# chto/linna

Measured on AMD Instinct MI355X. Metric: emulator log-likelihood evals/sec, higher is better.
Workload: dtype f32; 1 GPU; 33-D Gaussian, 4x512 MLP emulator (33->512x4->33), nwalkers=4096 batched log-likelihood per GPU (BASELINE configs[1]); nwalkers_per_gpu=4096, launch=direct launches, parallelism=walkers sharded, 1 rank(s), no data-path collective

## Files before the change

include/linna_hip.h:

```cpp
#ifndef LINNA_HIP_H
#define LINNA_HIP_H
#include <stddef.h>
#include <stdint.h>

#ifdef __cplusplus
extern "C" {
#endif

#define LINNA_ABI_VERSION 12

typedef struct linna_ctx linna_ctx_t;
typedef struct linna_net linna_net_t;
typedef struct linna_logprob linna_logprob_t;
typedef struct linna_graph linna_graph_t;

int linna_abi_version(void);
const char* linna_last_error(void);
#define LINNA_OK 0
#define LINNA_ERR_INVALID (-1)
#define LINNA_ERR_HIP (-2)
#define LINNA_ERR_UNSUPPORTED (-3)
#define LINNA_ERR_INTERNAL (-4)
int linna_debug_raise(int kind);
int linna_ctx_create(int device, linna_ctx_t** out);
// ... 129 lines not shown
                         linna_logprob_t** out);
int linna_logprob_destroy(linna_logprob_t* lp);
int linna_weights_changed(linna_ctx_t* ctx);
#define LINNA_PRECISION_FP32 0
#define LINNA_PRECISION_BF16 1
int linna_logprob_set_precision(linna_logprob_t* lp, int precision);
int linna_logprob_precision(const linna_logprob_t* lp, int* out);
int linna_logprob_set_grad_precision(linna_logprob_t* lp, int precision);
int linna_logprob_grad_precision(const linna_logprob_t* lp, int* out);
int linna_logprob_set_dense_grad(linna_logprob_t* lp, int on);
int linna_logprob_dense_grad(const linna_logprob_t* lp, int* out);
int linna_engine_rows(int rows);
int linna_dense_tri(int mode);
int linna_serve_plain(int on);
int linna_serve_plain_sched(int hand);
int linna_program_plain(const linna_layer_t* layers, int nlayers, int in_size, int rows, int dense_nout);
int linna_logprob_serve_plain(linna_logprob_t* lp, int B, int* out);
int linna_logprob_grad_launches(linna_logprob_t* lp, int B, int* out);
int linna_slice_fusion(int mask);
int linna_program_describe(const linna_layer_t* layers, int nlayers, int in_size, int rows, int dense_nout, char* buf,
                           size_t n);
int linna_program_describe_grad_bf16(const linna_layer_t* layers, int nlayers, int in_size, int rows, char* buf, size_t n);
int linna_program_describe_grad_dense(const linna_layer_t* layers, int nlayers, int in_size, int nout, int tri, int rows,
                                      char* buf, size_t n);
size_t linna_logprob_ws_bytes(const linna_logprob_t* lp, int B, int with_grad);
int linna_logprob_eval(linna_logprob_t* lp, const float* Z, int ldz, int B, void* ws, float* lnP,
                       float* THETA, int ldt, void* stream);
int linna_logprob_eval_if(linna_logprob_t* lp, const float* Z, int ldz, int B, void* ws, float* lnP,
                          float* THETA, int ldt, const int* gate, void* stream);
int linna_logprob_eval_slice_points(linna_logprob_t* lp, const float* coords, int ldc, int ndim, const int* S_idx,
// ... 196 lines not shown
```

linna_amd/_lib.py:

```python
import ctypes as C
import os

import torch

_HERE = os.path.dirname(os.path.abspath(__file__))
LIB_PATH = os.environ.get("LINNA_LIB_PATH") or os.path.join(_HERE, "liblinna_hip.so")
ABI_VERSION = 12
RHAT_BLOCK = 128

c_float_p = C.c_void_p
c_int_p = C.c_void_p


class _Sized(C.Structure):

    def __init__(self, *a, **k):
        C.Structure.__init__(self, *a, **k)
        self.struct_size = C.sizeof(type(self))


def sized_array(cls, n):
    arr = (cls * n)()
    for i in range(n):
        arr[i].struct_size = C.sizeof(cls)
# ... 95 lines not shown
    "linna_gauss_loglike_diag": (_I, [_V, _V, _I, _I, _I, _V, _V, _I, _I, _F, _V, _V]),
    "linna_gauss_loglike_dense": (_I, [_V, _V, _I, _I, _I, _V, _I, _V, _I, _I, _F, _V, _V, _V]),
    "linna_logprob_create": (_I, [_V, _V, C.POINTER(LogprobDesc), _PV]),
    "linna_logprob_destroy": (_I, [_V]),
    "linna_weights_changed": (_I, [_V]),
    "linna_logprob_set_precision": (_I, [_V, _I]),
    "linna_logprob_precision": (_I, [_V, _V]),
    "linna_logprob_set_grad_precision": (_I, [_V, _I]),
    "linna_logprob_grad_precision": (_I, [_V, _V]),
    "linna_logprob_set_dense_grad": (_I, [_V, _I]),
    "linna_logprob_dense_grad": (_I, [_V, _V]),
    "linna_engine_rows": (_I, [_I]),
    "linna_dense_tri": (_I, [_I]),
    "linna_serve_plain": (_I, [_I]),
    "linna_serve_plain_sched": (_I, [_I]),
    "linna_program_plain": (_I, [_V, _I, _I, _I, _I]),
    "linna_logprob_serve_plain": (_I, [_V, _I, _V]),
    "linna_logprob_grad_launches": (_I, [_V, _I, _V]),
    "linna_slice_fusion": (_I, [_I]),
    "linna_net_train_launches": (_I, [_V, _I]),
    "linna_net_set_train_precision": (_I, [_V, _I]),
    "linna_net_train_precision": (_I, [_V, _V]),
    "linna_program_describe": (_I, [_V, _I, _I, _I, _I, _V, C.c_size_t]),
    "linna_program_describe_grad_bf16": (_I, [_V, _I, _I, _I, _V, C.c_size_t]),
    "linna_program_describe_grad_dense": (_I, [_V, _I, _I, _I, _I, _I, _V, C.c_size_t]),
    "linna_logprob_ws_bytes": (_SZ, [_V, _I, _I]),
    "linna_logprob_eval": (_I, [_V, _V, _I, _I, _V, _V, _V, _I, _V]),
    "linna_logprob_grad": (_I, [_V, _V, _I, _I, _V, _V, _V, _I, _V]),
    "linna_logprob_grad_leapfrog": (_I, [_V, _V, _I, _I, _V, _V, _V, _I, _V, _I, _V, _F, _F, _V]),
    "linna_loss_scratch_bytes": (_SZ, [_I, _I]),
# ... 199 lines not shown

def slice_fusion(mask=-1):
    prev = load().linna_slice_fusion(int(mask))
    if prev < 0:
        check(prev)
    return prev


def serve_plain_sched(hand=-1):
    prev = load().linna_serve_plain_sched(int(hand))
    if prev < 0:
        check(prev)
    return prev


def serve_plain(on=-1):
    prev = load().linna_serve_plain(int(on))
    if prev < 0:
        check(prev)
    return prev


def engine_rows(rows=0):
    prev = load().linna_engine_rows(int(rows))
    if prev < 0:
        check(prev)
    return prev
```

linna_amd/csrc/api.hip:

```cpp
#include "common.h"

#include <stdarg.h>
#include <stdio.h>
#include <string.h>
#include <cstring>
#include <string>
#include <vector>
#include <atomic>
#include <new>
#include <stdlib.h>

namespace linna {

static thread_local std::string g_err;

void set_error(const char* fmt, ...) {
    char buf[512];
    va_list ap;
    va_start(ap, fmt);
    vsnprintf(buf, sizeof buf, fmt, ap);
    va_end(ap);
    g_err = buf;
}

// ... 1121 lines not shown
    static float dummy;
    if (dense_nout == -1) return net_stream_describe(ns_grad_kind(layers, nlayers), layers, nlayers, in_size, nullptr, rows, buf, n);
    const int dn_cols = dense_nout < -1 ? -dense_nout : dense_nout;
    NsDense dn{&dummy, (dn_cols + 3) & ~3, nullptr, nullptr, dense_nout < -1 ? 1 : 0, net_stream_dense_tri(-1)};
    if (dn_cols > 0) return net_stream_describe(NS_SERVE_DENSE, layers, nlayers, in_size, &dn, rows, buf, n);
    return net_stream_describe(NS_SERVE, layers, nlayers, in_size, nullptr, rows, buf, n);
} LINNA_CATCH_INT
int linna_serve_plain(int on) try {
    if (on < -1 || on > 1) { set_error("linna_serve_plain: %d (-1 query, 0 or 1)", on); return LINNA_ERR_INVALID; }
    return net_stream_serve_plain(on);
} LINNA_CATCH_INT
int linna_serve_plain_sched(int hand) try {
    if (hand < -1 || hand > 1) { set_error("linna_serve_plain_sched: %d (-1 query, 0 or 1)", hand); return LINNA_ERR_INVALID; }
    return net_stream_serve_plain_sched(hand);
} LINNA_CATCH_INT
int linna_program_plain(const linna_layer_t* layers, int nlayers, int in_size, int rows, int dense_nout) try {
    if (!layers || nlayers < 1) { set_error("program_plain: bad arguments"); return LINNA_ERR_INVALID; }
    TRY(check_layers(layers, nlayers, "program_plain"));
    if (dense_nout != 0) return 0;
    return net_stream_program_plain(NS_SERVE, layers, nlayers, in_size, nullptr, rows) ? 1 : 0;
} LINNA_CATCH_INT
int linna_logprob_serve_plain(linna_logprob_t* lp, int B, int* out) try {
    if (!lp || !out || B < 1) { set_error("logprob_serve_plain: bad arguments"); return LINNA_ERR_INVALID; }
    static float lnP;
    *out = lp_eval_route(lp, false).route == LP_EVAL_ONE &&
           net_stream_takes_plain(lp->kind(), net_layers(lp->net, lp->kind()), lp_output(lp), NsRun{nullptr, 0, B, &lnP}, nullptr, nullptr,
                                  net_stream_rows(B), nullptr);
    return LINNA_OK;
} LINNA_CATCH_INT
int linna_dense_tri(int mode) try {
// ... 740 lines not shown
```

linna_amd/csrc/common.h:

```cpp
#pragma once
#include <hip/hip_runtime.h>
#include <stdint.h>
#include <exception>
#include "../../include/linna_hip.h"


typedef float f32x4 __attribute__((ext_vector_type(4)));
typedef float f32x16 __attribute__((ext_vector_type(16)));

namespace linna {

struct U4 { uint32_t x, y, z, w; };
__device__ __forceinline__ U4 philox4x32_10(U4 c, uint32_t k0, uint32_t k1) {
#pragma unroll
    for (int r = 0; r < 10; ++r) {
        const uint64_t p0 = (uint64_t)0xD2511F53u * c.x;
        const uint64_t p1 = (uint64_t)0xCD9E8D57u * c.z;
        U4 n;
        n.x = (uint32_t)(p1 >> 32) ^ c.y ^ k0;
        n.y = (uint32_t)p1;
        n.z = (uint32_t)(p0 >> 32) ^ c.w ^ k1;
        n.w = (uint32_t)p0;
        c = n;
        k0 += 0x9E3779B9u; k1 += 0xBB67AE85u;
// ... 280 lines not shown
    NS_GRAD_INPUT_DENSE,
};
inline bool ns_kind_full_layers(NsKind k) { return k == NS_SERVE || k == NS_SERVE_DENSE || k == NS_SERVE_BF16; }
struct NsPlan { bool ok; size_t packed_floats; bool grad_ok; const char* why; };
NsPlan net_stream_plan(NsKind kind, const linna_layer_t* layers, int nl, int in_size, const NsDense* dn = nullptr);
int net_stream_rows(int B);
int net_stream_force_rows(int rows);
inline NsKind ns_grad_kind(const linna_layer_t* layers, int nl) { return nl >= 1 && layers[nl - 1].N > 64 ? NS_GRAD_INPUT_WIDE : NS_GRAD_INPUT; }
bool net_stream_grad_fits(const linna_layer_t* layers, int nl, int in_size, int rows);
bool net_stream_grad_dense_fits(const linna_layer_t* layers, int nl, int in_size, const NsDense* dn, int rows);
int launch_net_stream_pack(NsKind kind, const linna_layer_t* layers, int nl, int in_size, float* packed, int rows, const NsDense* dn,
                           hipStream_t s);
int net_stream_describe(NsKind kind, const linna_layer_t* layers, int nl, int in_size, const NsDense* dn, int rows, char* buf, size_t n);
int net_stream_serve_plain(int on);
int net_stream_serve_plain_sched(int hand);
bool net_stream_program_plain(NsKind kind, const linna_layer_t* layers, int nl, int in_size, const NsDense* dn, int rows);
bool net_stream_launch_plain_ok(bool cscale, bool cshift, bool w, bool cexp, bool lnP, bool D, bool TH, bool gate);
struct NsNet { const linna_layer_t* layers; int nl, in_size; };
struct NsInput { int nin; const int* is_flat; const float* a1; const float* a2; const int* lg; const float* xmean; const float* xstd; };
struct NsOutput { const float* cscale; const float* cshift; const float* cpost; const float* cshift2; const float* w; float T; };
struct NsRun { const float* Z; int ldz; int B; float* lnP; const int* gate = nullptr; float* TH = nullptr; int ldt = 0; float* D = nullptr; int ldd = 0; };
struct NsOpBufs { float* y; int ldy; float* t; int ldt; const float* x; int ldx; const float* gate; float* dprev; int ldp; float* dt; int lddt; };
struct NsPost { const float* rows; int n; float scale; float* out; int* step; float* hyper; float b1, b2; };
int launch_net_stream_dx(const NsNet& net, const float* packed, const float* dOUT, int lddo, int B, const NsOpBufs* ops, int with_input,
                         int rows, hipStream_t s, const NsPost* post = nullptr);
struct NsMove {
    float* coords; int ldc; float* logp; const int* S;
    const float* cc; int ldcc; const int* C; int nc;
    unsigned long long seed; const int* step; int step_off; int stream; float a; int* naccept;
    int slice;
// ... 98 lines not shown
```

linna_amd/csrc/net_program.hip:

```cpp
#include "net_program.h"
#include <stdlib.h>
#include <algorithm>
#include <atomic>
#include <cstring>
#include <mutex>
#include <string>
#include <unordered_map>

namespace linna {

size_t NsProgram::lds_for(int rows, bool grad) const {
    size_t b = (size_t)(2 * rows * LD + ((bias_total + 3) & ~3)) * sizeof(float) + 128 + (x0_keep ? 4096 : 0);
#ifdef NS_STAMPS
    b += NS_NW * 32 * 8;
#endif
    return b + (grad ? (size_t)mask_slots * 64 * NS_NW * sizeof(unsigned) : 0);
}

static int ceil16(int k) { return (k + 15) & ~15; }
int ns_seg_steps(const NsSeg& s) {
    if (s.type == NS_WIDE && s.zext < 0) return 2 * s.steps - 60;
    return s.type == NS_WIDE && s.zext > 0 ? s.steps + (s.passes - 1) * s.zext : s.steps * s.passes;
}
static int ns_switch(std::atomic<int>& sw, const char* name, int dflt, bool (*valid)(int)) {
// ... 399 lines not shown
        if (g.type != NS_WIDE && g.type != NS_SPLIT) return false;
        if (g.x0_col || (g.type == NS_WIDE && (g.zext || g.kslice))) return false;
    }
    return true;
}
bool net_stream_program_plain(NsKind kind, const linna_layer_t* layers, int nl, int in_size, const NsDense* dn, int rows) {
    return kind == NS_SERVE && rows == 16 && ns_program_plain(*ns_program(kind, layers, nl, in_size, dn, rows));
}
bool net_stream_launch_plain_ok(bool cscale, bool cshift, bool w, bool cexp, bool lnP, bool D, bool TH, bool gate) {
    return cscale && cshift && w && !cexp && lnP && !D && !TH && !gate;
}
static std::atomic<int> g_serve_plain{1};
int net_stream_serve_plain(int on) { return on < 0 ? g_serve_plain.load() : g_serve_plain.exchange(on ? 1 : 0); }
static std::atomic<int> g_serve_plain_sched{1};
int net_stream_serve_plain_sched(int hand) { return hand < 0 ? g_serve_plain_sched.load() : g_serve_plain_sched.exchange(hand ? 1 : 0); }

int ns_seg_cols(const NsProgram& p, const linna_layer_t* layers, int i) {
    if (p.seg_op[i] >= p.nops) return p.nout;
    const linna_layer_t& l = layers[p.seg_op[i]];
    return p.seg_hidden[i] ? l.C : i < p.nseg_f ? l.N : l.K;
}
NsGates ns_gates(const NsProgram& p, const linna_layer_t* layers, int nl, int rows) {
    NsGates g;
    for (int i = 0; i < NS_SEGCAP; ++i) g.gbit[i] = g.mbit[i] = -1;
    for (int i = 0; i < p.nseg_f; ++i) {
        const int op = p.seg_op[i];
        if (op >= nl || (!p.seg_hidden[i] && op == nl - 1)) continue;
        g.gbit[i] = g.ncols;
        g.ncols += (ns_seg_cols(p, layers, i) + 63) & ~63;
    }
// ... 235 lines not shown
```

linna_amd/csrc/net_stream.hip:

```cpp
#include "net_program.h"
#include <stdlib.h>
#include <type_traits>
#include <cstring>
#include <algorithm>

namespace linna {

typedef __bf16 bf16x8 __attribute__((ext_vector_type(8)));
typedef short s16x4 __attribute__((ext_vector_type(4)));

#ifndef NS_R
#define NS_R 6
#endif
#ifndef NS_PRE
#define NS_PRE 2
#endif
struct NsArgs {
    const float* Z; int ldz; int B; int nin;
    const int* is_flat; const float* a1; const float* a2; const int* lg;
    const float* xmean; const float* xstd;
    const float* packed;
    int G, nseg, LD, kpad0, nout, bias_total;
    int Gstride, nseg_f;
    const float* gscale; float* Gout; int ldg;
    float* hm_p; int hm_ldp; float* hm_q; const float* hm_mass; float hm_ek, hm_ed;
    const float* cscale; const float* cshift; const float* w; float T;
    const float* cpost; const float* cshift2;
    float* lnP; float* D; int ldd; float* TH; int ldt;
    unsigned long long* stamps;
    const int* gate;
    float* gout[NS_SEGCAP]; int gld[NS_SEGCAP]; int gn[NS_SEGCAP];
// ... 179 lines not shown
    constexpr int MOVE = 0, STORE = 0, ROWS = 16;
    constexpr bool GRAD = false, BF = false, EPS = false, PLAIN = true, WOUT = false, DGR = false;
#include "net_stream_body.inc"
}
#if NS_R == 6
#define NS_HAVE_PLACED 1
template <int R>
__global__ __launch_bounds__(64 * NS_NW, 1) void net_stream_placed_kernel(NsArgs a) {
    constexpr int MOVE = 0, STORE = 0, ROWS = 16;
    constexpr bool GRAD = false, BF = false, EPS = false, PLAIN = true, WOUT = false, DGR = false;
#define NS_BODY_HAND
#include "net_stream_body.inc"
#undef NS_BODY_HAND
}
#endif
template <int R, int MOVE, bool GRAD, int STORE, int ROWS, bool BF>
__global__ __launch_bounds__(64 * NS_NW, 1) void net_stream_train_bf16_kernel(NsArgs a) {
    static_assert(BF && GRAD && STORE == 3 && ROWS == 4 && MOVE == 0, "the bf16 training step only");
    constexpr bool EPS = false, PLAIN = false, WOUT = false, DGR = false;
#include "net_stream_body.inc"
}
template <int R, int MOVE, bool GRAD, int STORE, int ROWS, bool BF>
__global__ __launch_bounds__(64 * NS_NW, 1) void net_stream_slice_bf16_kernel(NsArgs a) {
    static_assert(BF && !GRAD && STORE == 0 && MOVE == 2, "the bf16 slice evaluation only");
    constexpr bool EPS = false, PLAIN = false, WOUT = false, DGR = false;
#define NS_BODY_SLICE_BF16
#include "net_stream_body.inc"
#undef NS_BODY_SLICE_BF16
}
template <int R, int MOVE, bool GRAD, int STORE, int ROWS, bool BF>
// ... 46 lines not shown
        }
        for (int ps = 0; ps < p.seg[i].passes; ++ps) {
            a.run_seg[nrun] = i; a.run_pass[nrun] = ps; a.run_first[nrun] = first;
            first += (ps > 0 && p.seg[i].type == NS_WIDE && p.seg[i].zext > 0) ? p.seg[i].zext : p.seg[i].steps; ++nrun;
        }
    }
    a.run_first[nrun] = first; a.nrun = nrun;
    const size_t total = (size_t)NS_NW * p.Gstride * NS_NT * 64 + (size_t)p.bias_total;
    hipLaunchKernelGGL(ns_pack_kernel, dim3((unsigned)((total + 255) / 256)), dim3(256), 0, s, a);
    if (p.side_f4) hipLaunchKernelGGL(ns_pack_side_kernel, dim3((unsigned)((p.side_f4 + 255) / 256)), dim3(256), 0, s, a);
    return check_hip(hipGetLastError(), "net_stream pack launch");
}

typedef void (*NsKernel)(NsArgs);
enum NsVariant { NV_SERVE, NV_STRETCH, NV_SLICE, NV_GRAD_MLP, NV_GRAD2, NV_STORE, NV_DX, NV_TRAIN_FWD, NV_TRAIN_STEP };
enum : unsigned { NF_BF16 = 1, NF_EPS = 2, NF_WIDE = 4, NF_PLAIN = 8, NF_PLACED = 16, NF_DENSE = 32 };
struct NsEntry { NsVariant v; unsigned flags; NsKernel k[3]; const char* what; const char* stamps_lacks; bool attr_set[3]; };
#define NS_ENGINES(K, MOVE, GRAD, STORE, ...) \
    {K<NS_R, MOVE, GRAD, STORE, 16, __VA_ARGS__>, K<NS_R, MOVE, GRAD, STORE, 8, __VA_ARGS__>, K<NS_R, MOVE, GRAD, STORE, 4, __VA_ARGS__>}
static NsEntry ns_table[] = {
    {NV_SERVE, 0, NS_ENGINES(net_stream_kernel, 0, false, 0, false), "net_stream launch"},
    {NV_SERVE, NF_BF16, NS_ENGINES(net_stream_kernel, 0, false, 0, true), "net_stream launch"},
    {NV_SERVE, NF_PLAIN, {net_stream_plain_kernel<NS_R>, nullptr, nullptr}, "net_stream plain launch"},
#ifdef NS_HAVE_PLACED
    {NV_SERVE, NF_PLAIN | NF_PLACED, {net_stream_placed_kernel<NS_R>, nullptr, nullptr}, "net_stream plain launch (hand-placed step)"},
#endif
    {NV_STRETCH, 0, NS_ENGINES(net_stream_kernel, 1, false, 0, false), "net_stream launch"},
    {NV_STRETCH, NF_BF16, NS_ENGINES(net_stream_kernel, 1, false, 0, true), "net_stream launch"},
    {NV_SLICE, 0, NS_ENGINES(net_stream_kernel, 2, false, 0, false), "net_stream launch"},
    {NV_SLICE, NF_BF16, NS_ENGINES(net_stream_slice_bf16_kernel, 2, false, 0, true), "net_stream bf16 slice launch", "bf16 slice evaluation"},
    {NV_GRAD_MLP, 0, NS_ENGINES(net_stream_kernel, 0, true, 0, false), "net_stream launch"},
    {NV_GRAD_MLP, NF_EPS, NS_ENGINES(net_stream_eps_kernel, 0, true, 0, false), "net_stream launch"},
    {NV_GRAD2, 0, NS_ENGINES(net_stream_kernel, 0, true, 2, false), "net_stream launch"},
    {NV_GRAD2, NF_EPS, NS_ENGINES(net_stream_eps_kernel, 0, true, 2, false), "net_stream launch"},
    {NV_GRAD2, NF_WIDE, NS_ENGINES(net_stream_wide_kernel, 0, true, 2, false, false), "net_stream wide-output gradient launch"},
    {NV_GRAD2, NF_WIDE | NF_EPS, NS_ENGINES(net_stream_wide_kernel, 0, true, 2, false, true), "net_stream wide-output gradient launch"},
    {NV_GRAD2, NF_DENSE, NS_ENGINES(net_stream_dense_kernel, 0, true, 2, false, false), "net_stream dense-covariance gradient launch"},
    {NV_GRAD2, NF_DENSE | NF_EPS, NS_ENGINES(net_stream_dense_kernel, 0, true, 2, false, true), "net_stream dense-covariance gradient launch"},
    {NV_GRAD2, NF_BF16, NS_ENGINES(net_stream_grad_bf16_kernel, 0, true, 2, true), "net_stream bf16 gradient launch", "bf16 gradient"},
    {NV_GRAD2, NF_BF16 | NF_EPS, NS_ENGINES(net_stream_eps_bf16_kernel, 0, true, 2, true), "net_stream bf16 gradient launch", "bf16 gradient"},
// ... 226 lines not shown
        a.mv_seed = mv->seed; a.mv_step = mv->step; a.mv_step_off = mv->step_off; a.mv_stream = mv->stream; a.mv_a = mv->a; a.mv_naccept = mv->naccept;
        a.mv_chain = mv->chain; a.mv_lps = mv->lps;
        a.sl_Z0 = mv->sl_Z0; a.sl_L = mv->sl_L; a.sl_R = mv->sl_R; a.sl_Zt = mv->sl_Zt; a.sl_m = mv->sl_m; a.sl_nt = mv->sl_nt;
        a.sl_seed = mv->sl_seed; a.sl_step = mv->sl_step; a.sl_stream = mv->sl_stream; a.sl_flags = mv->sl_flags;
        if (mv->sb) a.sb = *mv->sb;
        return ns_launch_program(mv->slice ? NV_SLICE : NV_STRETCH, fbf, a, r.B, p, rows, s);
    }
    if (bf && gr) { set_error("net_stream: no bf16 gradient"); return LINNA_ERR_UNSUPPORTED; }
    if (bf) return ns_launch_program(NV_SERVE, NF_BF16, a, r.B, p, rows, s);
    if (gr) {
        ns_set_grad(a, *gr);
        return ns_launch_program(NV_GRAD_MLP, a.hm_p && a.hm_eps ? NF_EPS : 0, a, r.B, p, rows, s);
    }
    if (!net_stream_takes_plain(kind, net, out, r, mv, gr, rows, dn)) return ns_launch_program(NV_SERVE, 0, a, r.B, p, rows, s);
    for (int i = 0; i < a.nseg; ++i) a.seg[i].type |= a.seg[i].ncg_log2 << 8;
#ifdef NS_HAVE_PLACED
    if (net_stream_serve_plain_sched(-1)) return ns_launch_program(NV_SERVE, NF_PLAIN | NF_PLACED, a, r.B, p, rows, s);
#endif
    return ns_launch_program(NV_SERVE, NF_PLAIN, a, r.B, p, rows, s);
}

int launch_net_stream_store(const NsNet& net, const float* packed, const float* X, int ldx, int B, const NsOpBufs* ops,
                            const float* cscale, const float* cshift, int rows, hipStream_t s) {
    const NsProgramRef pref = ns_program(NS_STORE, net.layers, net.nl, net.in_size, nullptr, rows);
    const NsProgram& p = *pref;
    if (!p.ok) { set_error("net_stream: network not eligible"); return LINNA_ERR_UNSUPPORTED; }
    NsArgs a = ns_args(p, packed, X, ldx, B, net.in_size, false);
    ns_set_input_ignored(a, X);
    a.cscale = cscale; a.cshift = cshift;
    ns_store_table(a, p, net, ops, 0, p.nseg_f, false);
// ... 106 lines not shown
```

linna_amd/csrc/net_stream_body.inc:

```
    constexpr int NT = NS_NT, NW = NS_NW;
    constexpr int RG = 32;
    constexpr bool SM = ROWS < 16;
    constexpr int RS = SM ? ROWS / 4 : 1;
    constexpr int NQ = SM ? RS : NT;
    constexpr int NACC = SM ? 4 * RS : NT;
#ifdef NS_BODY_SLICE_BF16
    static_assert(BF && !GRAD && STORE == 0 && MOVE == 2, "bf16: the slice evaluation");
#elif defined(NS_BODY_GRAD_BF16)
    static_assert(BF && GRAD && STORE == 2 && MOVE == 0, "bf16: lnP and its gradient in one launch");
#else
    static_assert(!BF || (!GRAD && STORE == 0 && MOVE != 2) || (GRAD && STORE == 3 && MOVE == 0 && ROWS == 4),
                  "bf16: serving, the fused stretch move and the merged training step (4-row engine)");
#endif
    constexpr bool BFT = BF && GRAD && STORE == 3;
    constexpr int AK = BF ? 2 : 1;
    constexpr bool K4 = !SM && !BF && (STORE == 0 || (GRAD && STORE == 2));
    constexpr bool TRB = GRAD && STORE == 3;
    constexpr bool DXE = STORE == 2 || TRB;
    constexpr bool G2 = GRAD && STORE == 2;
    constexpr bool LB = G2;
    constexpr bool LATE_REFILL = true;
#ifdef NS_BODY_HAND
    constexpr bool HAND = true;
    static_assert(PLAIN && !BF && ROWS == 16 && R == 6 && NS_NT == 4 && LATE_REFILL, "the hand-placed step: plain fp32 serving, 16 rows, six slots");
#else
    constexpr bool HAND = false;
#endif
#define NS_HAND_RING \
    "+{v[128:131]}"(Bq[0][0]), "+{v[132:135]}"(Bq[0][1]), "+{v[136:139]}"(Bq[0][2]), "+{v[140:143]}"(Bq[0][3]), \
    "+{v[144:147]}"(Bq[1][0]), "+{v[148:151]}"(Bq[1][1]), "+{v[152:155]}"(Bq[1][2]), "+{v[156:159]}"(Bq[1][3]), \
    "+{v[160:163]}"(Bq[2][0]), "+{v[164:167]}"(Bq[2][1]), "+{v[168:171]}"(Bq[2][2]), "+{v[172:175]}"(Bq[2][3]), \
    "+{v[176:179]}"(Bq[3][0]), "+{v[180:183]}"(Bq[3][1]), "+{v[184:187]}"(Bq[3][2]), "+{v[188:191]}"(Bq[3][3]), \
    "+{v[192:195]}"(Bq[4][0]), "+{v[196:199]}"(Bq[4][1]), "+{v[200:203]}"(Bq[4][2]), "+{v[204:207]}"(Bq[4][3]), \
    "+{v[208:211]}"(Bq[5][0]), "+{v[212:215]}"(Bq[5][1]), "+{v[216:219]}"(Bq[5][2]), "+{v[220:223]}"(Bq[5][3])
#define NS_HAND_A "+{v[224:227]}"(Aq[0][0]), "+{v[228:231]}"(Aq[1][0])
#define NS_HAND_ACC "+{v[232:235]}"(acc[0]), "+{v[236:239]}"(acc[1]), "+{v[240:243]}"(acc[2]), "+{v[244:247]}"(acc[3])
    constexpr bool RNAN = STORE == 1;
    auto relu_f = [](float v) { if constexpr (RNAN) return isnan(v) ? v : fmaxf(v, 0.f); else return fmaxf(v, 0.f); };
    static_assert(ROWS == 16 || ROWS == 8 || ROWS == 4, "rows per workgroup");
    static_assert(R % 2 == 0, "the A double buffer alternates with the ring slot parity");
    extern __shared__ __attribute__((aligned(16))) float smem[];
// ... 309 lines not shown
                asm volatile("global_store_dword %0, %1, off" :: "v"(a.t_xb + (size_t)(row0 + pr) * a.t_ldxb + c), "v"(x) : "memory");
        }
        if constexpr (BF) {
            if (prow) {
                if (c < nin) { const float hi = (float)(__bf16)x; act[pr * LD + c] = hi; act[pr * LD + nin + c] = x - hi; }
                else if (c >= 2 * nin) act[pr * LD + c] = 0.f;
            }
        } else {
            if (prow) act[pr * LD + c] = x;
        }
    }
    __builtin_amdgcn_sched_barrier(0);
#ifdef NS_STAMPS_FINE
    NS_STAMP();
#endif
    NS_PF_ALL(PRE, (LATE_REFILL ? R - 1 : R))
#undef NS_PF_ALL
#undef NS_PF
#pragma unroll
    for (int o = RG / 2; o >= 1; o >>= 1) zz += __shfl_xor(zz, o, 64);
#pragma unroll
    for (int i = 0; i < BMAX; ++i) {
        const int j = tid + i * 64 * NW;
        if (j < nb4) reinterpret_cast<f32x4*>(lbias)[j] = breg[i];
    }
    int* const lsrc = reinterpret_cast<int*>(lbias + ((a.bias_total + 3) & ~3));
    float* const lden = reinterpret_cast<float*>(lsrc + 16);
    if constexpr (STORE == 3) {
        if (prow && pc0 == 0) { lsrc[pr] = zsrc; lden[pr] = zden; }
    }
    float* const lx0 = lden + 16;
// ... 1 lines not shown
    if (a.x0_keep && prow) {
#pragma unroll
        for (int i = 0; i < ZPRE; ++i) {
            const int c = pc0 + i * RG;
            if constexpr (BF) lx0[pr * 64 + c] = c < nin ? act[pr * LD + c] + act[pr * LD + nin + c] : 0.f;
            else lx0[pr * 64 + c] = (c < kpad0) ? act[pr * LD + c] : 0.f;
        }
    }
    }
    asm volatile("s_waitcnt lgkmcnt(0)" ::: "memory");
    __builtin_amdgcn_s_barrier();
    asm volatile("" ::: "memory");
    NS_STAMP();

    if constexpr (HAND) {
#pragma unroll
        for (int t = 0; t < NT; ++t) Bq[R - 1][t] = f32x4{0.f, 0.f, 0.f, 0.f};
        asm volatile("" : NS_HAND_RING :: "memory");
    }
    const uint32_t act_lds = (uint32_t)(uintptr_t)(__attribute__((address_space(3))) void*)act;
    f32x4 acc[NACC];
    f32x4 Aq[2][AK];
    const int sm_arow = (4 * ((lane >> 2) & 3) + (lane & 3)) % ROWS, sm_achunk = lane >> 4;
    int si = 0, pass = 0, P = 0, kleft;
    int s_type, s_steps, s_passes, s_bias, s_dst, s_relu, s_kslice, s_zext, s_ncgl, s_mstore = 0, s_mapply = 0, s_x0col = 0, s_x0n = 0, s_kcl = 0;
    unsigned* const lmask = reinterpret_cast<unsigned*>(lbias + ((a.bias_total + 3) & ~3));
    float lnp_grad = 0.f;
    float* s_gout = nullptr; int s_gld = 0, s_gn = 0;
    const float* s_gmask = nullptr; int s_gmld = 0;
    int s_gbit = -1, s_mbit = -1;
    auto gstore = [&](float* p, float v) { asm volatile("global_store_dword %0, %1, off" :: "v"(p), "v"(v) : "memory"); };
    uint32_t ap;
// ... 52 lines not shown
    auto lds_barrier = [&]() {
        asm volatile("s_waitcnt lgkmcnt(0)" ::: "memory");
        __builtin_amdgcn_s_barrier();
        asm volatile("" ::: "memory");
    };
    if constexpr (PLAIN) {
        asm volatile("" :: "s"(seg_warm));
        plain_take(ka->seg[0]); begin_run(); a_read(Aq[0]); plain_request();
    }
    else {
    load_seg();
    begin_run();
    a_read(Aq[0]);
    }

    auto step = [&](auto Uc, auto Refill) {
        constexpr int U = decltype(Uc)::value;
        constexpr bool refill = decltype(Refill)::value;
        constexpr int RU = LATE_REFILL ? (U + R - 1) % R : U;
        if constexpr (HAND) {
            constexpr int BU = 128 + 16 * U, BR = 128 + 16 * RU, AC = 224 + 4 * (U & 1), AN = 224 + 4 * ((U + 1) & 1);
            constexpr int TW = refill ? 0 : 4 * U;
#define NS_HM(t, s) "v_mfma_f32_16x16x4_f32 v[232+4*" #t ":235+4*" #t "], v[%[ac]+" #s "], v[%[bu]+4*" #t "+" #s "], v[232+4*" #t ":235+4*" #t "]\n\t"
#define NS_HL(t, off) "global_load_dwordx4 v[%[ru]+4*" #t ":%[ru]+4*" #t "+3], %[vo], %[sb] offset:" #off "\n\t"
#define NS_HAND_TEXT(HEAD, L0, L1, L2, L3) HEAD \
            "s_waitcnt lgkmcnt(0)\n\t" \
            "s_waitcnt vmcnt(%[w0])\n\t" \
            NS_HM(0, 0) "ds_read_b128 v[%[an]:%[an]+3], %[ap]\n\t" \
            "s_waitcnt vmcnt(%[w1])\n\t" \
            NS_HM(1, 0) \
            NS_HM(0, 1) L0 \
            NS_HM(1, 1) \
            NS_HM(0, 2) L1 \
            NS_HM(1, 2) \
            NS_HM(0, 3) L2 \
            NS_HM(1, 3) \
            "s_waitcnt vmcnt(%[w2])\n\t" \
            NS_HM(2, 0) L3 \
            "s_waitcnt vmcnt(%[w3])\n\t" \
            NS_HM(3, 0) \
            NS_HM(2, 1) "v_add_u32 %[ap], 64, %[ap]\n\t" \
            NS_HM(3, 1) NS_HM(2, 2) NS_HM(3, 2) NS_HM(2, 3) NS_HM(3, 3)
            if constexpr (refill) {
                const char* const sb = wbase + woff;
#ifdef NS_HAND_PHASE4
#define NS_HAND_HEAD ".p2align 3\n\ts_nop 0\n\t"
#else
#define NS_HAND_HEAD ".p2align 3\n\t"
#endif
                if constexpr (U == 0)
                    asm volatile(NS_HAND_TEXT(NS_HAND_HEAD, NS_HL(0, 0), NS_HL(1, 1024), NS_HL(2, 2048), NS_HL(3, 3072))
                                 : NS_HAND_RING, NS_HAND_A, NS_HAND_ACC, [ap] "+v"(ap)
                                 : [vo] "v"(voff), [sb] "s"(sb), [bu] "n"(BU), [ru] "n"(BR), [ac] "n"(AC), [an] "n"(AN),
                                   [w0] "n"(19), [w1] "n"(18), [w2] "n"(20), [w3] "n"(20) : "memory");
                else
                    asm volatile(NS_HAND_TEXT("", NS_HL(0, 0), NS_HL(1, 1024), NS_HL(2, 2048), NS_HL(3, 3072))
                                 : NS_HAND_RING, NS_HAND_A, NS_HAND_ACC, [ap] "+v"(ap)
                                 : [vo] "v"(voff), [sb] "s"(sb), [bu] "n"(BU), [ru] "n"(BR), [ac] "n"(AC), [an] "n"(AN),
                                   [w0] "n"(19), [w1] "n"(18), [w2] "n"(20), [w3] "n"(20) : "memory");
                wadvance();
            } else {
                asm volatile(NS_HAND_TEXT("", "", "", "", "")
                             : NS_HAND_RING, NS_HAND_A, NS_HAND_ACC, [ap] "+v"(ap)
                             : [bu] "n"(BU), [ac] "n"(AC), [an] "n"(AN),
                               [w0] "n"(19 - TW), [w1] "n"(18 - TW), [w2] "n"(17 - TW), [w3] "n"(16 - TW) : "memory");
            }
#undef NS_HAND_TEXT
#undef NS_HAND_HEAD
#undef NS_HL
#undef NS_HM
        } else {
        if constexpr (BF) asm volatile("s_waitcnt lgkmcnt(0)" : "+v"(Aq[U & 1][0]), "+v"(Aq[U & 1][AK - 1]) :: "memory");
        else asm volatile("s_waitcnt lgkmcnt(0)" : "+v"(Aq[U & 1][0]) :: "memory");
        a_read(Aq[(U + 1) & 1]);
        const f32x4 av = Aq[U & 1][0];
        if constexpr (BF) {
            bf16x8 ab;
#pragma unroll
            for (int e = 0; e < 4; ++e) { ab[e] = (__bf16)Aq[U & 1][0][e]; ab[4 + e] = (__bf16)Aq[U & 1][AK - 1][e]; }
            if constexpr (SM) {
                auto bf_small = [&]() {
                    const s16x4 alo = __builtin_bit_cast(s16x4, __builtin_shufflevector(ab, ab, 0, 1, 2, 3));
                    const s16x4 ahi = __builtin_bit_cast(s16x4, __builtin_shufflevector(ab, ab, 4, 5, 6, 7));
// ... 597 lines not shown
                    take_seg(N2);
                    if constexpr (LB) { s_gbit = ka->gbit[n2i]; s_mbit = ka->mbit[n2i]; s_gn = ka->gn[n2i]; }
                }
            }
            if (si < nseg) {
                begin_run();
                a_read(Aq[(U + 1) & 1]);
                if constexpr (PLAIN) { if (seg_done) plain_request(); }
            }
#ifdef NS_STAMPS_FINE
            if (fine) { asm volatile("s_waitcnt lgkmcnt(0)" ::: "memory"); NS_STAMP(); }
#endif
        }
    };
    using T_ = std::true_type; using F_ = std::false_type;
#define NS_STEP(U, RF) if constexpr (U < R) step(std::integral_constant<int, U>{}, RF{});
    const int ngroups = a.G / R, rem = a.G - ngroups * R;
#pragma unroll 1
    for (int it = 0; it < ngroups; ++it) {
        NS_STEP(0, T_) NS_STEP(1, T_) NS_STEP(2, T_) NS_STEP(3, T_) NS_STEP(4, T_) NS_STEP(5, T_) NS_STEP(6, T_) NS_STEP(7, T_)
    }
#define NS_TAIL(U) if constexpr (U < R - 1) { if (rem > U) step(std::integral_constant<int, U>{}, F_{}); }
    NS_TAIL(0) NS_TAIL(1) NS_TAIL(2) NS_TAIL(3) NS_TAIL(4) NS_TAIL(5) NS_TAIL(6)
#undef NS_STEP
#undef NS_TAIL
    if constexpr (BF) asm volatile("s_waitcnt lgkmcnt(0)" : "+v"(Aq[0][0]), "+v"(Aq[0][AK - 1]), "+v"(Aq[1][0]), "+v"(Aq[1][AK - 1]) :: "memory");
    else asm volatile("s_waitcnt lgkmcnt(0)" : "+v"(Aq[0][0]), "+v"(Aq[1][0]) :: "memory");
    NS_STAMP();

    if constexpr (((STORE == 1 || STORE == 2) && !GRAD) || TRB) { NS_STAMPS_FLUSH(); return; }
    if constexpr (STORE == 3) {
        const float* const F = act + P * ABUF + pr * LD;
        const bool rok = prow && row0 + pr < a.B;
        const float* const Dv = a.u_same ? F : act + (P ^ 1) * ABUF + pr * LD;
        const float* const Uv = a.u_same ? F + a.u_col : F;
        float chi = 0.f;
        for (int c = pc0; c < nout; c += RG) chi += Dv[c] * Uv[c];
#pragma unroll
// ... 125 lines not shown
```

Before: 76.52 million evals/s.

## Ramp the weight-prefetch ring in the hand-placed plain serving kernel head

```diff
diff --git a/include/linna_hip.h b/include/linna_hip.h
--- a/include/linna_hip.h
+++ b/include/linna_hip.h
@@ -167,6 +167,7 @@
 int linna_dense_tri(int mode);
 int linna_serve_plain(int on);
 int linna_serve_plain_sched(int hand);
+int linna_serve_head(int ramp);
 int linna_program_plain(const linna_layer_t* layers, int nlayers, int in_size, int rows, int dense_nout);
 int linna_logprob_serve_plain(linna_logprob_t* lp, int B, int* out);
 int linna_logprob_grad_launches(linna_logprob_t* lp, int B, int* out);
diff --git a/linna_amd/_lib.py b/linna_amd/_lib.py
--- a/linna_amd/_lib.py
+++ b/linna_amd/_lib.py
@@ -133,6 +133,7 @@
     "linna_dense_tri": (_I, [_I]),
     "linna_serve_plain": (_I, [_I]),
     "linna_serve_plain_sched": (_I, [_I]),
+    "linna_serve_head": (_I, [_I]),
     "linna_program_plain": (_I, [_V, _I, _I, _I, _I]),
     "linna_logprob_serve_plain": (_I, [_V, _I, _V]),
     "linna_logprob_grad_launches": (_I, [_V, _I, _V]),
@@ -362,6 +363,13 @@
     return prev
 
 
+def serve_head(ramp=-1):
+    prev = load().linna_serve_head(int(ramp))
+    if prev < 0:
+        check(prev)
+    return prev
+
+
 def serve_plain(on=-1):
     prev = load().linna_serve_plain(int(on))
     if prev < 0:
diff --git a/linna_amd/csrc/api.hip b/linna_amd/csrc/api.hip
--- a/linna_amd/csrc/api.hip
+++ b/linna_amd/csrc/api.hip
@@ -1159,6 +1159,10 @@
     if (hand < -1 || hand > 1) { set_error("linna_serve_plain_sched: %d (-1 query, 0 or 1)", hand); return LINNA_ERR_INVALID; }
     return net_stream_serve_plain_sched(hand);
 } LINNA_CATCH_INT
+int linna_serve_head(int ramp) try {
+    if (ramp < -1 || ramp > 1) { set_error("linna_serve_head: %d (-1 query, 0 or 1)", ramp); return LINNA_ERR_INVALID; }
+    return net_stream_serve_head(ramp);
+} LINNA_CATCH_INT
 int linna_program_plain(const linna_layer_t* layers, int nlayers, int in_size, int rows, int dense_nout) try {
     if (!layers || nlayers < 1) { set_error("program_plain: bad arguments"); return LINNA_ERR_INVALID; }
     TRY(check_layers(layers, nlayers, "program_plain"));
diff --git a/linna_amd/csrc/common.h b/linna_amd/csrc/common.h
--- a/linna_amd/csrc/common.h
+++ b/linna_amd/csrc/common.h
@@ -318,6 +318,7 @@
 int net_stream_describe(NsKind kind, const linna_layer_t* layers, int nl, int in_size, const NsDense* dn, int rows, char* buf, size_t n);
 int net_stream_serve_plain(int on);
 int net_stream_serve_plain_sched(int hand);
+int net_stream_serve_head(int ramp);
 bool net_stream_program_plain(NsKind kind, const linna_layer_t* layers, int nl, int in_size, const NsDense* dn, int rows);
 bool net_stream_launch_plain_ok(bool cscale, bool cshift, bool w, bool cexp, bool lnP, bool D, bool TH, bool gate);
 struct NsNet { const linna_layer_t* layers; int nl, in_size; };
diff --git a/linna_amd/csrc/net_program.hip b/linna_amd/csrc/net_program.hip
--- a/linna_amd/csrc/net_program.hip
+++ b/linna_amd/csrc/net_program.hip
@@ -437,6 +437,8 @@
 int net_stream_serve_plain(int on) { return on < 0 ? g_serve_plain.load() : g_serve_plain.exchange(on ? 1 : 0); }
 static std::atomic<int> g_serve_plain_sched{1};
 int net_stream_serve_plain_sched(int hand) { return hand < 0 ? g_serve_plain_sched.load() : g_serve_plain_sched.exchange(hand ? 1 : 0); }
+static std::atomic<int> g_serve_head{1};
+int net_stream_serve_head(int ramp) { return ramp < 0 ? g_serve_head.load() : g_serve_head.exchange(ramp ? 1 : 0); }
 
 int ns_seg_cols(const NsProgram& p, const linna_layer_t* layers, int i) {
     if (p.seg_op[i] >= p.nops) return p.nout;
diff --git a/linna_amd/csrc/net_stream.hip b/linna_amd/csrc/net_stream.hip
--- a/linna_amd/csrc/net_stream.hip
+++ b/linna_amd/csrc/net_stream.hip
@@ -15,6 +15,22 @@
 #ifndef NS_PRE
 #define NS_PRE 2
 #endif
+#define NS_RAMP_STEPS 3
+constexpr int ns_ring_slots(int pre, int ramped, int tail) { return pre + ramped - tail; }
+constexpr int ns_ring_vmcnt(int pre, int ramped, int tail, int issued, int t) { return 4 * ns_ring_slots(pre, ramped, tail) - 1 - t + issued; }
+static_assert((ns_ring_vmcnt(NS_R - 1, 0, 0, 0, 0) == 19 && ns_ring_vmcnt(NS_R - 1, 0, 0, 0, 1) == 18 &&
+               ns_ring_vmcnt(NS_R - 1, 0, 0, 3, 2) == 20 && ns_ring_vmcnt(NS_R - 1, 0, 0, 4, 3) == 20) || NS_R != 6, "steady step");
+static_assert((ns_ring_vmcnt(NS_PRE, NS_RAMP_STEPS, 0, 0, 0) == 19 && ns_ring_vmcnt(NS_PRE, NS_RAMP_STEPS, 0, 0, 1) == 18 &&
+               ns_ring_vmcnt(NS_PRE, NS_RAMP_STEPS, 0, 3, 2) == 20 && ns_ring_vmcnt(NS_PRE, NS_RAMP_STEPS, 0, 4, 3) == 20) || NS_R != 6 || NS_PRE != 2,
+              "steady step behind the ramp");
+constexpr bool ns_ring_tail_ok(int pre, int ramped) {
+    for (int u = 0; u < 5; ++u)
+        for (int t = 0; t < 4; ++t)
+            if (ns_ring_vmcnt(pre, ramped, u, 0, t) != 19 - 4 * u - t) return false;
+    return true;
+}
+static_assert((ns_ring_tail_ok(NS_R - 1, 0) && ns_ring_tail_ok(NS_PRE, NS_RAMP_STEPS)) || NS_R != 6 || NS_PRE != 2, "tail steps");
+static_assert((4 * ns_ring_slots(NS_PRE, 0, 0) == 8 && 4 * ns_ring_slots(NS_PRE, NS_RAMP_STEPS, 0) == 20) || NS_R != 6 || NS_PRE != 2, "ramp");
 struct NsArgs {
     const float* Z; int ldz; int B; int nin;
     const int* is_flat; const float* a1; const float* a2; const int* lg;
@@ -224,6 +240,19 @@
 #undef NS_BODY_HAND
 }
 #endif
+#if NS_R == 6 && NS_PRE == 2
+#define NS_HAVE_RAMP 1
+template <int R>
+__global__ __launch_bounds__(64 * NS_NW, 1) void net_stream_ramp_kernel(NsArgs a) {
+    constexpr int MOVE = 0, STORE = 0, ROWS = 16;
+    constexpr bool GRAD = false, BF = false, EPS = false, PLAIN = true, WOUT = false, DGR = false;
+#define NS_BODY_HAND
+#define NS_BODY_RAMP
+#include "net_stream_body.inc"
+#undef NS_BODY_RAMP
+#undef NS_BODY_HAND
+}
+#endif
 template <int R, int MOVE, bool GRAD, int STORE, int ROWS, bool BF>
 __global__ __launch_bounds__(64 * NS_NW, 1) void net_stream_train_bf16_kernel(NsArgs a) {
     static_assert(BF && GRAD && STORE == 3 && ROWS == 4 && MOVE == 0, "the bf16 training step only");
@@ -300,7 +329,7 @@
 
 typedef void (*NsKernel)(NsArgs);
 enum NsVariant { NV_SERVE, NV_STRETCH, NV_SLICE, NV_GRAD_MLP, NV_GRAD2, NV_STORE, NV_DX, NV_TRAIN_FWD, NV_TRAIN_STEP };
-enum : unsigned { NF_BF16 = 1, NF_EPS = 2, NF_WIDE = 4, NF_PLAIN = 8, NF_PLACED = 16, NF_DENSE = 32 };
+enum : unsigned { NF_BF16 = 1, NF_EPS = 2, NF_WIDE = 4, NF_PLAIN = 8, NF_PLACED = 16, NF_DENSE = 32, NF_RAMP = 64 };
 struct NsEntry { NsVariant v; unsigned flags; NsKernel k[3]; const char* what; const char* stamps_lacks; bool attr_set[3]; };
 #define NS_ENGINES(K, MOVE, GRAD, STORE, ...) \
     {K<NS_R, MOVE, GRAD, STORE, 16, __VA_ARGS__>, K<NS_R, MOVE, GRAD, STORE, 8, __VA_ARGS__>, K<NS_R, MOVE, GRAD, STORE, 4, __VA_ARGS__>}
@@ -310,6 +339,9 @@
     {NV_SERVE, NF_PLAIN, {net_stream_plain_kernel<NS_R>, nullptr, nullptr}, "net_stream plain launch"},
 #ifdef NS_HAVE_PLACED
     {NV_SERVE, NF_PLAIN | NF_PLACED, {net_stream_placed_kernel<NS_R>, nullptr, nullptr}, "net_stream plain launch (hand-placed step)"},
+#endif
+#ifdef NS_HAVE_RAMP
+    {NV_SERVE, NF_PLAIN | NF_PLACED | NF_RAMP, {net_stream_ramp_kernel<NS_R>, nullptr, nullptr}, "net_stream plain launch (hand-placed step, ramped head)"},
 #endif
     {NV_STRETCH, 0, NS_ENGINES(net_stream_kernel, 1, false, 0, false), "net_stream launch"},
     {NV_STRETCH, NF_BF16, NS_ENGINES(net_stream_kernel, 1, false, 0, true), "net_stream launch"},
@@ -566,6 +598,9 @@
     }
     if (!net_stream_takes_plain(kind, net, out, r, mv, gr, rows, dn)) return ns_launch_program(NV_SERVE, 0, a, r.B, p, rows, s);
     for (int i = 0; i < a.nseg; ++i) a.seg[i].type |= a.seg[i].ncg_log2 << 8;
+#ifdef NS_HAVE_RAMP
+    if (net_stream_serve_plain_sched(-1) && net_stream_serve_head(-1)) return ns_launch_program(NV_SERVE, NF_PLAIN | NF_PLACED | NF_RAMP, a, r.B, p, rows, s);
+#endif
 #ifdef NS_HAVE_PLACED
     if (net_stream_serve_plain_sched(-1)) return ns_launch_program(NV_SERVE, NF_PLAIN | NF_PLACED, a, r.B, p, rows, s);
 #endif
diff --git a/linna_amd/csrc/net_stream_body.inc b/linna_amd/csrc/net_stream_body.inc
--- a/linna_amd/csrc/net_stream_body.inc
+++ b/linna_amd/csrc/net_stream_body.inc
@@ -25,6 +25,12 @@
     static_assert(PLAIN && !BF && ROWS == 16 && R == 6 && NS_NT == 4 && LATE_REFILL, "the hand-placed step: plain fp32 serving, 16 rows, six slots");
 #else
     constexpr bool HAND = false;
+#endif
+#ifdef NS_BODY_RAMP
+    constexpr bool RAMP = true;
+    static_assert(HAND && NS_PRE == 2 && NS_PRE + NS_RAMP_STEPS == R - 1, "the ramp: two slots from the prologue, five after three steps");
+#else
+    constexpr bool RAMP = false;
 #endif
 #define NS_HAND_RING \
     "+{v[128:131]}"(Bq[0][0]), "+{v[132:135]}"(Bq[0][1]), "+{v[136:139]}"(Bq[0][2]), "+{v[140:143]}"(Bq[0][3]), \
@@ -364,7 +370,7 @@
 #ifdef NS_STAMPS_FINE
     NS_STAMP();
 #endif
-    NS_PF_ALL(PRE, (LATE_REFILL ? R - 1 : R))
+    NS_PF_ALL(PRE, (RAMP ? PRE : LATE_REFILL ? R - 1 : R))
 #undef NS_PF_ALL
 #undef NS_PF
 #pragma unroll
@@ -396,8 +402,15 @@
     NS_STAMP();
 
     if constexpr (HAND) {
+        if constexpr (RAMP) {
+            asm volatile("" : "={v[160:163]}"(Bq[2][0]), "={v[164:167]}"(Bq[2][1]), "={v[168:171]}"(Bq[2][2]), "={v[172:175]}"(Bq[2][3]),
+                              "={v[176:179]}"(Bq[3][0]), "={v[180:183]}"(Bq[3][1]), "={v[184:187]}"(Bq[3][2]), "={v[188:191]}"(Bq[3][3]),
+                              "={v[192:195]}"(Bq[4][0]), "={v[196:199]}"(Bq[4][1]), "={v[200:203]}"(Bq[4][2]), "={v[204:207]}"(Bq[4][3]),
+                              "={v[208:211]}"(Bq[5][0]), "={v[212:215]}"(Bq[5][1]), "={v[216:219]}"(Bq[5][2]), "={v[220:223]}"(Bq[5][3]));
+        } else {
 #pragma unroll
         for (int t = 0; t < NT; ++t) Bq[R - 1][t] = f32x4{0.f, 0.f, 0.f, 0.f};
+        }
         asm volatile("" : NS_HAND_RING :: "memory");
     }
     const uint32_t act_lds = (uint32_t)(uintptr_t)(__attribute__((address_space(3))) void*)act;
@@ -480,16 +493,24 @@
     a_read(Aq[0]);
     }
 
-    auto step = [&](auto Uc, auto Refill) {
+    auto step = [&](auto Uc, auto Refill, auto Xc) {
         constexpr int U = decltype(Uc)::value;
         constexpr bool refill = decltype(Refill)::value;
+        constexpr int X = decltype(Xc)::value; (void)X;
         constexpr int RU = LATE_REFILL ? (U + R - 1) % R : U;
         if constexpr (HAND) {
-            constexpr int BU = 128 + 16 * U, BR = 128 + 16 * RU, AC = 224 + 4 * (U & 1), AN = 224 + 4 * ((U + 1) & 1);
-            constexpr int TW = refill ? 0 : 4 * U;
+            constexpr bool ramp = RAMP && refill && X >= 0;
+            static_assert(!ramp || (X == U && X < NS_RAMP_STEPS), "ramp steps are the launch's first");
+            constexpr int BU = 128 + 16 * U, BR = 128 + 16 * (ramp ? (2 * X + 2) % R : RU), AC = 224 + 4 * (U & 1), AN = 224 + 4 * ((U + 1) & 1);
+            constexpr int BR2 = 128 + 16 * ((2 * X + 3 + R) % R);
+            constexpr int VP = RAMP ? PRE : R - 1;
+            constexpr int VG = !RAMP ? 0 : ramp ? X : NS_RAMP_STEPS;
+            constexpr int VT = refill ? 0 : X;
+            static_assert(ramp || !refill || ns_ring_slots(VP, VG, VT) == R - 1, "steady state: five slots in flight");
 #define NS_HM(t, s) "v_mfma_f32_16x16x4_f32 v[232+4*" #t ":235+4*" #t "], v[%[ac]+" #s "], v[%[bu]+4*" #t "+" #s "], v[232+4*" #t ":235+4*" #t "]\n\t"
 #define NS_HL(t, off) "global_load_dwordx4 v[%[ru]+4*" #t ":%[ru]+4*" #t "+3], %[vo], %[sb] offset:" #off "\n\t"
-#define NS_HAND_TEXT(HEAD, L0, L1, L2, L3) HEAD \
+#define NS_HL2(t, off) "global_load_dwordx4 v[%[r2]+4*" #t ":%[r2]+4*" #t "+3], %[vo], %[s2] offset:" #off "\n\t"
+#define NS_HAND_TEXT(HEAD, L0, L1, L2, L3, L4, L5, L6, L7) HEAD \
             "s_waitcnt lgkmcnt(0)\n\t" \
             "s_waitcnt vmcnt(%[w0])\n\t" \
             NS_HM(0, 0) "ds_read_b128 v[%[an]:%[an]+3], %[ap]\n\t" \
@@ -504,35 +525,50 @@
             "s_waitcnt vmcnt(%[w2])\n\t" \
             NS_HM(2, 0) L3 \
             "s_waitcnt vmcnt(%[w3])\n\t" \
-            NS_HM(3, 0) \
+            NS_HM(3, 0) L4 \
             NS_HM(2, 1) "v_add_u32 %[ap], 64, %[ap]\n\t" \
-            NS_HM(3, 1) NS_HM(2, 2) NS_HM(3, 2) NS_HM(2, 3) NS_HM(3, 3)
-            if constexpr (refill) {
+            NS_HM(3, 1) L5 NS_HM(2, 2) L6 NS_HM(3, 2) L7 NS_HM(2, 3) NS_HM(3, 3)
+            if constexpr (ramp) {
+                const char* const sb = wbase + woff;
+                wadvance();
+                const char* const s2 = wbase + woff;
+                wadvance();
+                asm volatile(NS_HAND_TEXT("", NS_HL(0, 0), NS_HL(1, 1024), NS_HL(2, 2048), NS_HL(3, 3072),
+                                          NS_HL2(0, 0), NS_HL2(1, 1024), NS_HL2(2, 2048), NS_HL2(3, 3072))
+                             : NS_HAND_RING, NS_HAND_A, NS_HAND_ACC, [ap] "+v"(ap)
+                             : [vo] "v"(voff), [sb] "s"(sb), [s2] "s"(s2), [bu] "n"(BU), [ru] "n"(BR), [r2] "n"(BR2), [ac] "n"(AC), [an] "n"(AN),
+                               [w0] "n"(ns_ring_vmcnt(VP, VG, VT, 0, 0)), [w1] "n"(ns_ring_vmcnt(VP, VG, VT, 0, 1)),
+                               [w2] "n"(ns_ring_vmcnt(VP, VG, VT, 3, 2)), [w3] "n"(ns_ring_vmcnt(VP, VG, VT, 4, 3)) : "memory");
+            } else if constexpr (refill) {
                 const char* const sb = wbase + woff;
 #ifdef NS_HAND_PHASE4
 #define NS_HAND_HEAD ".p2align 3\n\ts_nop 0\n\t"
 #else
 #define NS_HAND_HEAD ".p2align 3\n\t"
 #endif
-                if constexpr (U == 0)
-                    asm volatile(NS_HAND_TEXT(NS_HAND_HEAD, NS_HL(0, 0), NS_HL(1, 1024), NS_HL(2, 2048), NS_HL(3, 3072))
+                if constexpr (U == (RAMP ? NS_RAMP_STEPS : 0))
+                    asm volatile(NS_HAND_TEXT(NS_HAND_HEAD, NS_HL(0, 0), NS_HL(1, 1024), NS_HL(2, 2048), NS_HL(3, 3072), "", "", "", "")
                                  : NS_HAND_RING, NS_HAND_A, NS_HAND_ACC, [ap] "+v"(ap)
                                  : [vo] "v"(voff), [sb] "s"(sb), [bu] "n"(BU), [ru] "n"(BR), [ac] "n"(AC), [an] "n"(AN),
-                                   [w0] "n"(19), [w1] "n"(18), [w2] "n"(20), [w3] "n"(20) : "memory");
+                                   [w0] "n"(ns_ring_vmcnt(VP, VG, VT, 0, 0)), [w1] "n"(ns_ring_vmcnt(VP, VG, VT, 0, 1)),
+                                   [w2] "n"(ns_ring_vmcnt(VP, VG, VT, 3, 2)), [w3] "n"(ns_ring_vmcnt(VP, VG, VT, 4, 3)) : "memory");
                 else
-                    asm volatile(NS_HAND_TEXT("", NS_HL(0, 0), NS_HL(1, 1024), NS_HL(2, 2048), NS_HL(3, 3072))
+                    asm volatile(NS_HAND_TEXT("", NS_HL(0, 0), NS_HL(1, 1024), NS_HL(2, 2048), NS_HL(3, 3072), "", "", "", "")
                                  : NS_HAND_RING, NS_HAND_A, NS_HAND_ACC, [ap] "+v"(ap)
                                  : [vo] "v"(voff), [sb] "s"(sb), [bu] "n"(BU), [ru] "n"(BR), [ac] "n"(AC), [an] "n"(AN),
-                                   [w0] "n"(19), [w1] "n"(18), [w2] "n"(20), [w3] "n"(20) : "memory");
+                                   [w0] "n"(ns_ring_vmcnt(VP, VG, VT, 0, 0)), [w1] "n"(ns_ring_vmcnt(VP, VG, VT, 0, 1)),
+                                   [w2] "n"(ns_ring_vmcnt(VP, VG, VT, 3, 2)), [w3] "n"(ns_ring_vmcnt(VP, VG, VT, 4, 3)) : "memory");
                 wadvance();
             } else {
-                asm volatile(NS_HAND_TEXT("", "", "", "", "")
+                asm volatile(NS_HAND_TEXT("", "", "", "", "", "", "", "", "")
                              : NS_HAND_RING, NS_HAND_A, NS_HAND_ACC, [ap] "+v"(ap)
                              : [bu] "n"(BU), [ac] "n"(AC), [an] "n"(AN),
-                               [w0] "n"(19 - TW), [w1] "n"(18 - TW), [w2] "n"(17 - TW), [w3] "n"(16 - TW) : "memory");
+                               [w0] "n"(ns_ring_vmcnt(VP, VG, VT, 0, 0)), [w1] "n"(ns_ring_vmcnt(VP, VG, VT, 0, 1)),
+                               [w2] "n"(ns_ring_vmcnt(VP, VG, VT, 0, 2)), [w3] "n"(ns_ring_vmcnt(VP, VG, VT, 0, 3)) : "memory");
             }
 #undef NS_HAND_TEXT
 #undef NS_HAND_HEAD
+#undef NS_HL2
 #undef NS_HL
 #undef NS_HM
         } else {
@@ -1160,14 +1196,29 @@
         }
     };
     using T_ = std::true_type; using F_ = std::false_type;
-#define NS_STEP(U, RF) if constexpr (U < R) step(std::integral_constant<int, U>{}, RF{});
+#define NS_STEP(U, RF) if constexpr (U < R) step(std::integral_constant<int, U>{}, RF{}, std::integral_constant<int, -1>{});
+#define NS_TAIL(U) if constexpr (U < R - 1) { if (rem > U) step(std::integral_constant<int, U>{}, F_{}, std::integral_constant<int, U>{}); }
     const int ngroups = a.G / R, rem = a.G - ngroups * R;
+    if constexpr (RAMP) {
+#define NS_RAMP(U) if (nhead > U) step(std::integral_constant<int, U>{}, T_{}, std::integral_constant<int, U>{});
+#define NS_RTAIL(K) if (rrem > K) step(std::integral_constant<int, (NS_RAMP_STEPS + K) % R>{}, F_{}, std::integral_constant<int, K>{});
+        const int nhead = min(a.G, NS_RAMP_STEPS);
+        const int rgroups = (a.G - nhead) / R, rrem = (a.G - nhead) - rgroups * R;
+        NS_RAMP(0) NS_RAMP(1) NS_RAMP(2)
+#pragma unroll 1
+        for (int it = 0; it < rgroups; ++it) {
+            NS_STEP(3, T_) NS_STEP(4, T_) NS_STEP(5, T_) NS_STEP(0, T_) NS_STEP(1, T_) NS_STEP(2, T_)
+        }
+        NS_RTAIL(0) NS_RTAIL(1) NS_RTAIL(2) NS_RTAIL(3) NS_RTAIL(4)
+#undef NS_RAMP
+#undef NS_RTAIL
+    } else {
 #pragma unroll 1
     for (int it = 0; it < ngroups; ++it) {
         NS_STEP(0, T_) NS_STEP(1, T_) NS_STEP(2, T_) NS_STEP(3, T_) NS_STEP(4, T_) NS_STEP(5, T_) NS_STEP(6, T_) NS_STEP(7, T_)
     }
-#define NS_TAIL(U) if constexpr (U < R - 1) { if (rem > U) step(std::integral_constant<int, U>{}, F_{}); }
     NS_TAIL(0) NS_TAIL(1) NS_TAIL(2) NS_TAIL(3) NS_TAIL(4) NS_TAIL(5) NS_TAIL(6)
+    }
 #undef NS_STEP
 #undef NS_TAIL
     if constexpr (BF) asm volatile("s_waitcnt lgkmcnt(0)" : "+v"(Aq[0][0]), "+v"(Aq[0][AK - 1]), "+v"(Aq[1][0]), "+v"(Aq[1][AK - 1]) :: "memory");
```

Result: no change. 76.54 million evals/s (median of 2 runs) (+0.0%).
